# BenniG123/icp-slam-prototype

Hardware: AMD Instinct MI355X
Metric: ICP iterations/sec + NN Mpoints/sec at 307k-pt Kinect cloud, 1/2/4/8 GPU (higher is better)
Workload: dtype f32 filter + f64 exact pair arithmetic (reference float semantics), f64 reductions and solve; 1 GPU; kinect640x480_30pct: ONE frame pair, 91870 source x 92170 target points, 20 fixed ICP iterations per step from the pair's initial pose, solve=reference, nn=grid (BASELINE configs[1]); the N > 1 lines run configs[3] (64 such pairs) and scale against frame_batch (--full); parallelism=1 GPU

## Files before the change

icp_slam_prototype_amd/csrc/icpk_align.cpp:

```cpp
#include <chrono>
#include <cstring>
#include <utility>
#include <vector>

#include "icpk_ctx.h"
#include "solve_impl.h"

using namespace icpk;

namespace {

hipEvent_t get_event(icpk_ctx* ctx, size_t k) {
  while (ctx->events.size() <= k) {
    hipEvent_t e = nullptr;
    if (hipEventCreate(&e) != hipSuccess) return nullptr;
    ctx->events.push_back(e);
  }
  return ctx->events[k];
}

void log_delta(icpk_ctx* ctx, int key, int quantity) {
  if (!ctx->log_fn) return;
  const auto now = std::chrono::steady_clock::now();
  const double us = std::chrono::duration<double, std::micro>(now - ctx->log_last).count();
// ... 64 lines not shown

void pack_pose(float T_out[16], int solve, const float Trot[9], const float offset[3], const double Tk[12]) {
  if (solve == ICPK_SOLVE_REFERENCE) {
    for (int r = 0; r < 3; ++r) {
      for (int c = 0; c < 3; ++c) T_out[4 * r + c] = Trot[3 * r + c];
      T_out[4 * r + 3] = offset[r];
    }
  } else {
    for (int r = 0; r < 3; ++r)
      for (int c = 0; c < 4; ++c) T_out[4 * r + c] = (float)Tk[4 * r + c];
  }
  T_out[12] = T_out[13] = T_out[14] = 0.f;
  T_out[15] = 1.f;
}

int begin_alignment(icpk_ctx* ctx) {
  const int rc = copy_src0_to_src(ctx);
  if (rc) return rc;
  ctx->src_pristine = false;
  ctx->have_seed = false;
  ctx->have_qperm = false;
  clear_trace(ctx);
  return ICPK_OK;
}

}

namespace icpk {

int loop_nsum(const icpk_params* p) {
  if (p->solve == ICPK_SOLVE_POINT_TO_PLANE || p->solve == ICPK_SOLVE_PLANE_TO_PLANE) return NP2L;
  return p->solve == ICPK_SOLVE_REFERENCE ? NSUM_REF : NSUM;
}

int device_loop_begin(icpk_ctx* ctx, const icpk_params* p, bool throttled, bool mirror, bool defer) {
  LoopInitArgs a{};
  a.st = ctx->st_dev;
  if (throttled || mirror) {
    ctx->loop_epoch = (ctx->loop_epoch % 1000000) + 1;
    a.epoch = ctx->loop_epoch;
    a.progress = ctx->progress_dev;
    a.mirror = mirror ? ctx->st_mirror_dev : nullptr;
  }
  a.max_iterations = p->max_iterations;
  a.min_pairs = p->min_pairs;
  a.solve = p->solve;
  a.fixed_iterations = p->fixed_iterations;
  a.threshold = p->threshold;
  std::memcpy(a.last_rotation, p->last_rotation, sizeof(a.last_rotation));
  std::memcpy(a.last_translation, p->last_translation, sizeof(a.last_translation));
  if (defer) {
    ctx->pending_init = a;
    ctx->init_pending = true;
  } else {
    launch_loop_init(a, ctx->stream);
    ICPK_HIP(ctx, hipGetLastError());
  }
  const int nsum = loop_nsum(p);
// ... 156 lines not shown
  if (rc) return rc;
  if (!p || !T_out) return ICPK_E_ARG;
  if (p->nn_mode == ICPK_NN_MAP) return fail(ctx, ICPK_E_ARG, "ICPK_NN_MAP is single-context only");
  if (p->solve == ICPK_SOLVE_PLANE_TO_PLANE) return fail(ctx, ICPK_E_ARG, "the query-sharded loop has no plane-to-plane flavour");
  if (colored_step(ctx, p)) return fail(ctx, ICPK_E_ARG, "the query-sharded loop has no colored flavour (icpk_set_colored is on)");
  if (!ctx->comm) return fail(ctx, ICPK_E_NOT_SET, "icpk_comm_init_rccl has not been called");
  if (p->solve != ICPK_SOLVE_REFERENCE && p->solve != ICPK_SOLVE_KABSCH)
    return fail(ctx, ICPK_E_ARG, "the query-sharded loop supports the reference and Kabsch flavours");
  if (p->max_iterations < 0 || p->max_iterations > LOOP_MAX_ITER) return fail(ctx, ICPK_E_ARG, "max_iterations out of range");
  if (p->min_pairs < 1) return fail(ctx, ICPK_E_ARG, "min_pairs must be >= 1");
  if (ctx->robust_on) return fail(ctx, ICPK_E_ARG, "robust alignment is not available in the query-sharded loop");
  ICPK_HIP(ctx, hipSetDevice(ctx->device));
  reset_outputs(T_out, stats);
  icpk_params q = *p;
  q.nn_mode = ICPK_NN_GRID;
  rc = begin_alignment(ctx);
  if (rc) return rc;
  const LoopGuard guard{ctx};
  rc = device_loop_begin(ctx, &q, false);
  if (rc) return rc;
  ctx->loop_nact = NSUM;
  const int B = red_blocks(ctx->src.n);
  auto sweep = [&]() -> int {
    int r = enqueue_nn(ctx, ICPK_NN_GRID);
    if (r) return r;
    r = enqueue_reduce(ctx, q.max_nn_dist);
    if (r) return r;
    launch_reduce_final_shard(ctx->partial, ctx->pcount, B, ctx->red_out, ctx->st_dev, ctx->stream);
    return icpk_comm_allreduce_device(ctx, ctx->red_out, NSUM + 1);
  };
  rc = sweep();
// ... 28 lines not shown
  if (gicp && ctx->robust_on) return fail(ctx, ICPK_E_ARG, "plane-to-plane has no robust form (icpk_set_robust is on)");
  if (gicp && (!ctx->have_normals || !ctx->have_src_normals))
    return fail(ctx, ICPK_E_NOT_SET, "plane-to-plane needs source and target normals");
  const bool colored = colored_step(ctx, p);
  if (colored && ctx->robust_on) return fail(ctx, ICPK_E_ARG, "colored ICP has no robust form (icpk_set_robust is on)");
  if (colored && (!ctx->have_src_colors || !ctx->have_tgt_colors || !ctx->have_color_gradients))
    return fail(ctx, ICPK_E_NOT_SET, "colored ICP needs source colours, target colours and target colour gradients");
  if (ctx->robust_on && p->solve == ICPK_SOLVE_REFERENCE)
    return fail(ctx, ICPK_E_ARG, "robust alignment needs the Kabsch or point-to-plane flavour");
  int rc = check_ready(ctx);
  if (rc) {
    if (stats) stats->status = rc;
    return rc;
  }
  ICPK_HIP(ctx, hipSetDevice(ctx->device));
  rc = begin_alignment(ctx);
  if (rc) return rc;
  const bool robust = ctx->robust_on;
  if (robust && ctx->src.n > 0 && (rc = ensure_robust(ctx, ctx->src.n))) return rc;
  if (!p->host_loop && !ctx->log_fn && ctx->src.n > 0 && p->max_iterations <= LOOP_MAX_ITER)
    return align_device_loop(ctx, p, T_out, stats);

  Profiler pf(ctx, p);
  const bool p2l = p->solve == ICPK_SOLVE_POINT_TO_PLANE;
  const int nsum = robust ? (p2l ? NP2L_W : NSUM_W) : (p2l || gicp ? NP2L : NSUM);
  double Tk[12] = {1, 0, 0, 0, 0, 1, 0, 0, 0, 0, 1, 0};
  double sums[NSUM_MAX];
  int64_t npairs = 0, kept = 0;
  double wsum = 0.0;
  RobustSel sel{};
  float mse = 0.f;
  auto sweep = [&]() -> int {
    int r = pf.sweep(p->nn_mode);
    if (r) return r;
    r = pf.stamp(&pf.red);
    if (r) return r;
// ... 148 lines not shown
```

icp_slam_prototype_amd/csrc/icpk_api.cpp:

```cpp
#include <cmath>
#include <cstdlib>
#include <cstring>
#include <string>

#include "icpk_ctx.h"
#include "solve_impl.h"

using namespace icpk;

namespace {

int upload_cloud(icpk_ctx* ctx, Cloud& c, const float* x, const float* y, const float* z, int n, float pad,
                 hipMemcpyKind kind, bool sync = true) {
  if (n < 0 || (n > 0 && (!x || !y || !z))) return fail(ctx, ICPK_E_ARG, "bad cloud pointers/size");
  int rc = ensure_cloud(ctx, c, n);
  if (rc) return rc;
  if (n > 0 && kind == hipMemcpyHostToDevice && !sync) {
    PinnedBuf<float>& stage = (&c == &ctx->tgt) ? ctx->stage_t : ctx->stage_s;
    if ((rc = stage.reserve(ctx, (size_t)3 * c.cap))) return rc;
    std::memcpy(stage, x, (size_t)n * sizeof(float));
    std::memcpy(stage + c.cap, y, (size_t)n * sizeof(float));
    std::memcpy(stage + 2 * (size_t)c.cap, z, (size_t)n * sizeof(float));
    ICPK_HIP(ctx, hipMemcpyAsync(c.base, stage, ((size_t)2 * c.cap + n) * sizeof(float), hipMemcpyHostToDevice, ctx->stream));
  } else if (n > 0) {
// ... 121 lines not shown
  ICPK_HIP(ctx, hipSetDevice(ctx->device));
  int rc = upload_cloud(ctx, ctx->src0, x, y, z, n, 0.f, k, sync);
  if (rc) return rc;
  ctx->have_src = true;
  ctx->have_assoc = false;
  ctx->have_seed = false;
  ctx->have_qperm = false;
  return copy_src0_to_src(ctx);
}

int copy_src0_to_src(icpk_ctx* ctx) {
  ctx->rec_pending = false;
  if (ctx->src_pristine && ctx->tune.pristine_skip && ctx->src.n == ctx->src0.n) return ICPK_OK;
  int rc = ensure_cloud(ctx, ctx->src, ctx->src0.n);
  if (rc) return rc;
  const Cloud &a = ctx->src0, &b = ctx->src;
  if (a.cap == b.cap) {
    ICPK_HIP(ctx, hipMemcpyAsync(b.base, a.base, (size_t)3 * a.cap * sizeof(float), hipMemcpyDeviceToDevice, ctx->stream));
  } else {
    const int m = round_up(a.n < 1 ? 1 : a.n, NN_TILE);
    ICPK_HIP(ctx, hipMemcpyAsync(b.x(), a.x(), (size_t)m * sizeof(float), hipMemcpyDeviceToDevice, ctx->stream));
    ICPK_HIP(ctx, hipMemcpyAsync(b.y(), a.y(), (size_t)m * sizeof(float), hipMemcpyDeviceToDevice, ctx->stream));
    ICPK_HIP(ctx, hipMemcpyAsync(b.z(), a.z(), (size_t)m * sizeof(float), hipMemcpyDeviceToDevice, ctx->stream));
  }
  ctx->src_pristine = true;
  return ICPK_OK;
}

int check_ready(icpk_ctx* ctx) {
  if (!ctx) return ICPK_E_ARG;
  if (!ctx->have_tgt || !ctx->have_src) return fail(ctx, ICPK_E_NOT_SET, "source or target cloud not set");
  if (ctx->tgt.n <= 0) return fail(ctx, ICPK_E_EMPTY_TARGET, "target cloud is empty");
  return ICPK_OK;
}

int pad_target(icpk_ctx* ctx) {
  Cloud& c = ctx->tgt;
  const int padded = round_up(c.n < 1 ? 1 : c.n, NN_TILE);
  launch_fill_f32(c.x() + c.n, padded - c.n, __builtin_inff(), ctx->stream);
  launch_fill_f32(c.y() + c.n, padded - c.n, __builtin_inff(), ctx->stream);
// ... 306 lines not shown
```

icp_slam_prototype_amd/csrc/icpk_ctx.h:

```cpp
#pragma once
#include <hip/hip_runtime.h>

#include <chrono>
#include <string>
#include <thread>
#include <vector>

#include "icpk.h"
#include "icpk_internal.h"

struct icpk_ctx;

namespace icpk {

inline int hip_failure(icpk_ctx* ctx, const char* what, hipError_t e);

struct DeviceMem {
  static constexpr const char* name = "hipMalloc";
  static hipError_t alloc(void** p, size_t bytes) { return hipMalloc(p, bytes); }
  static hipError_t free(void* p) { return hipFree(p); }
};
template <unsigned Flags>
struct PinnedMem {
  static constexpr const char* name = "hipHostMalloc";
// ... 183 lines not shown
  int sub_factor = 0;
  unsigned long long sub_seed = 0;
  unsigned long long sub_stream = 0;
  struct HostRange {
    const char* host;
    size_t bytes;
    const char* dev;
  };
  std::vector<HostRange> registered;
  icpk::PinnedBuf<uint16_t> stage_depth;
  icpk::DevBuf<int> pix_tidx;
  icpk::DevBuf<int> pix_src;
  bool have_pix_seed = false;
  int pix_rows = 0, pix_cols = 0;
  bool src_pristine = false;
  const int* stop = nullptr;
  LoopState* st_active = nullptr;
  icpk::PinnedBuf<float> stage_t, stage_s;
  icpk::DevBuf<uint16_t> depth_dev;
  icpk::DevBuf<uint16_t> depth_flt;
  icpk::DevBuf<uint16_t> bil_tables;
  std::vector<uint16_t> bil_tables_host;
  icpk_bilateral_params bil_params = {0, 0.f, 0.f, 0};
  int bil_K = 0;
  icpk::DevBuf<int32_t> ks_buf;
  int frame_slot = -1;
  int frame_rows = 0, frame_cols = 0;
  int frame_filter[6] = {0, 0, 0, 0, 0, 0};
  icpk::DevBuf<int> bp_counts;
  icpk::PinnedBuf<int> bp_n_host;
// ... 186 lines not shown
    t_query = now + std::chrono::milliseconds(20);
    const hipError_t q = hipStreamQuery(stream ? stream : ctx->stream);
    if (q == hipSuccess) return done() ? ICPK_OK : fail(ctx, ICPK_E_HIP, stalled);
    if (q != hipErrorNotReady) return fail(ctx, ICPK_E_HIP, hipGetErrorString(q));
  }
  return ICPK_OK;
}

icpk_ctx* make_context(int device_id, const icpk_ctx* parent);
int check_ready(icpk_ctx* ctx);
int set_target_impl(icpk_ctx* ctx, const float* x, const float* y, const float* z, int32_t n, hipMemcpyKind k,
                    bool sync = true);
int set_source_impl(icpk_ctx* ctx, const float* x, const float* y, const float* z, int32_t n, hipMemcpyKind k,
                    bool sync = true);
int copy_src0_to_src(icpk_ctx* ctx);
int pad_target(icpk_ctx* ctx);
void target_changed(icpk_ctx* ctx, bool keep_normals);
void reset_outputs(float T_out[16], icpk_stats* stats);
void clear_trace(icpk_ctx* ctx);

int ensure_cloud(icpk_ctx* ctx, Cloud& c, int n);
int ensure_assoc(icpk_ctx* ctx, int nq);
int index_cloud(icpk_ctx* ctx, const float* x, const float* y, const float* z, int n, GridIndex& g);
int index_target(icpk_ctx* ctx, GridView* out);
int index_aux(icpk_ctx* ctx, const Cloud& c, GridView* out);
int ensure_unpacked(icpk_ctx* ctx);
int flush_loop_init(icpk_ctx* ctx);
NnArgs base_nn_args(const icpk_ctx* ctx);
int prepare_sorted_sweep(icpk_ctx* ctx, int nn_mode, NnArgs& a, NnBoxes& bx, int& recheck);
GridSweepArgs grid_sweep_args(icpk_ctx* ctx, const NnArgs& a, const NnBoxes& bx);
void after_grid_sweep(icpk_ctx* ctx);
int enqueue_nn(icpk_ctx* ctx, int nn_mode, hipEvent_t ev0 = nullptr, hipEvent_t ev1 = nullptr);
const float4* loop_rec(const icpk_ctx* ctx);
int enqueue_reduce(icpk_ctx* ctx, float max_dist);
int enqueue_reduce_p2l(icpk_ctx* ctx, float max_dist);
int enqueue_reduce_gicp(icpk_ctx* ctx, float max_dist, const float* R_acc);
int enqueue_reduce_colored(icpk_ctx* ctx, float max_dist);
inline bool colored_step(const icpk_ctx* ctx, const icpk_params* p) {
  return ctx->colored_on && p->solve == ICPK_SOLVE_POINT_TO_PLANE;
}
int ensure_robust(icpk_ctx* ctx, int nq);
// ... 18 lines not shown
```

icp_slam_prototype_amd/csrc/icpk_internal.h:

```cpp
#pragma once
#include <hip/hip_runtime.h>
#include <stddef.h>
#include <stdint.h>

#include "tsdf_rule.h"

namespace icpk {

constexpr int NN_THREADS = 256;
constexpr int NN_TILE = 1024;
static_assert(NN_TILE == 4 * NN_THREADS, "one float4 per lane per plane per tile");

typedef unsigned long long nn_key_t;
constexpr nn_key_t NN_KEY_INIT = ~0ull;

struct NnArgs {
  const float* qx;
  const float* qy;
  const float* qz;
  int nq;
  const float* tx;
  const float* ty;
  const float* tz;
  int nt_pad;
// ... 124 lines not shown
  int status;
  int sweeps;
  int steps;
  long long pairs;
  float mse;
  int epoch;
  int* progress;
  LoopState* mirror;
  Rt rt;
  double Rd[9];
  float Trot[9];
  float offset[3];
  double Tk[12];
  int max_iterations, min_pairs, solve, fixed_iterations;
  float threshold;
  float last_rotation[9], last_translation[3];
  float trace_R[LOOP_MAX_ITER * 9];
  float trace_t[LOOP_MAX_ITER * 3];
  float trace_mse[LOOP_MAX_ITER];
  int trace_pairs[LOOP_MAX_ITER];
};
__device__ __forceinline__ bool loop_stopped(const int* stop) { return stop && (stop[0] | stop[1]); }

struct StepArgs {
  const double* partial;
  const int* pcount;
  int nblocks;
  int pad0;
  LoopState* st;
};
// ... 176 lines not shown
  int n, n_pad;
  float pad;
  int cap1;
  float* d1;
  float* d2;
  int cap2;
  int pad0;
};
struct LoopInitArgs {
  LoopState* st;
  int* progress;
  LoopState* mirror;
  int max_iterations, min_pairs, solve, fixed_iterations;
  float threshold;
  int epoch;
  float last_rotation[9], last_translation[3];
};
struct BoundsArgs {
  const float *x, *y, *z;
  float* fb;
  int n, nparts;
};
struct InfoArgs {
  const float* fb;
  GridInfo* g;
  int nparts, n;
  float ppc;
  int xdiv;
  int max_cells;
  int pad0;
// ... 66 lines not shown
inline int grid_bounds_parts(int n) {
  const int nb = (n + 2047) / 2048;
  return nb < 1 ? 1 : (nb > GRID_BOUNDS_PARTS ? GRID_BOUNDS_PARTS : nb);
}
inline BoundsArgs bounds_args(const float* x, const float* y, const float* z, int n, float* fb) {
  return BoundsArgs{x, y, z, fb, n, grid_bounds_parts(n)};
}
inline InfoArgs info_args(const float* fb, int n, float ppc, int xdiv, int max_cells, GridInfo* g) {
  return InfoArgs{fb, g, grid_bounds_parts(n), n, ppc, xdiv < 1 ? 1 : xdiv, max_cells < 64 ? 64 : max_cells, 0};
}
void launch_ingest_cloud(const IngestArgs& a, hipStream_t s);
void launch_loop_init(const LoopInitArgs& a, hipStream_t s);
void launch_grid_bounds(const BoundsArgs& a, hipStream_t s);
void launch_grid_info(const InfoArgs& a, hipStream_t s);
void launch_grid_qslot(const QslotArgs& a, hipStream_t s);
void launch_grid_scan(const ScanArgs& a, hipStream_t s);
void launch_grid_tscatter(const TscatterArgs& a, hipStream_t s);
void launch_grid_qscatter(const QscatterArgs& a, hipStream_t s);
void launch_grid_begin(const BoundsArgs& a, const InfoArgs& info, const LoopInitArgs* init, int* ticket, hipStream_t s);
bool flush_setup_batches(const SetupRecorder* recs, int count, hipStream_t s);
void replay_setup(const SetupRecorder& rec, hipStream_t s);
void launch_ingest_batch(const SetupBatchOf<IngestArgs>& b, int count, hipStream_t s);
void launch_loop_init_batch(const SetupBatchOf<LoopInitArgs>& b, int count, hipStream_t s);
void launch_grid_bounds_batch(const SetupBatchOf<BoundsArgs>& b, int count, hipStream_t s);
void launch_grid_info_batch(const SetupBatchOf<InfoArgs>& b, int count, hipStream_t s);
void launch_grid_qslot_batch(const SetupBatchOf<QslotArgs>& b, int count, hipStream_t s);
void launch_grid_scan_batch(const SetupBatchOf<ScanArgs>& b, int count, hipStream_t s);
void launch_grid_tscatter_batch(const SetupBatchOf<TscatterArgs>& b, int count, hipStream_t s);
void launch_grid_qscatter_batch(const SetupBatchOf<QscatterArgs>& b, int count, hipStream_t s);
void launch_grid_tqscatter(const TscatterArgs& t, const QscatterArgs& q, hipStream_t s);
// ... 333 lines not shown
```

icp_slam_prototype_amd/csrc/icpk_sweep.cpp:

```cpp
#include <cstring>
#include <utility>

#include "icpk_ctx.h"

using namespace icpk;

namespace icpk {

int ensure_cloud(icpk_ctx* ctx, Cloud& c, int n) {
  if (ctx && (&c == &ctx->src0 || &c == &ctx->src)) ctx->src_pristine = false;
  if (ctx && &c == &ctx->src) ctx->rec_pending = false;
  if (ctx && &c == &ctx->src0) ctx->have_src_normals = false;
  if (ctx && &c == &ctx->src0) fpfh_dropped(ctx, 0);
  if (ctx && &c == &ctx->src0) ctx->have_src_colors = false;
  if (ctx && (&c == &ctx->src0 || &c == &ctx->tgt)) ctx->have_pix_seed = false;
  if (ctx && (&c == &ctx->src0 || &c == &ctx->tgt)) ctx->have_score_assoc = false;
  const int cap = round_up(n < 1 ? 1 : n, NN_TILE);
  if (cap > c.cap) {
    c.cap = 0;
    if (int rc = c.base.reserve(ctx, (size_t)3 * cap + 64)) return rc;
    c.cap = cap;
  }
  c.n = n;
  return ICPK_OK;
}

// ... 130 lines not shown
    ctx->have_grid = !rc;
  }
  if (!rc && out) *out = ctx->grid.view();
  return rc;
}

int index_aux(icpk_ctx* ctx, const Cloud& c, GridView* out) {
  if (c.n > (1 << 28)) return fail(ctx, ICPK_E_ARG, "the grid search addresses its cell-sorted points with 32-bit byte offsets: at most 2^28 points");
  int rc = ctx->aux_grid.reserve(ctx, c.n);
  if (!rc) rc = index_cloud(ctx, c.x(), c.y(), c.z(), c.n, ctx->aux_grid);
  if (!rc) *out = ctx->aux_grid.view();
  return rc;
}

static QscatterArgs query_scatter_args(icpk_ctx* ctx, const int* qcell, const int* qslot, float4* qm4, bool pix) {
  return QscatterArgs{qcell,        qslot,        ctx->qstart,  ctx->qperm, ctx->src.x(), ctx->src.y(), ctx->src.z(),
                      ctx->tgt.x(), ctx->tgt.y(), ctx->tgt.z(), qm4,        ctx->sp_in,   ctx->seed_m,  ctx->src.n,
                      0,            pix ? ctx->pix_src.get() : nullptr,     pix ? ctx->pix_tidx.get() : nullptr,
                      ctx->pix_rows, ctx->pix_cols};
}

static int enqueue_cell_order(icpk_ctx* ctx, bool with_points) {
  const int nq = ctx->src.n;
  int rc = ensure_sort_buffers(ctx, nq);
  if (rc) return rc;
  rc = ensure_scan_buffers(ctx);
  if (rc) return rc;
  int* qcell = reinterpret_cast<int*>(ctx->sort_keys + ctx->sort_cap);
  int* qslot = ctx->sort_vals;
  const bool ident = ctx->have_pix_seed && ctx->tune.image_order;
  const bool pix = ctx->have_pix_seed && ctx->tune.pixel_seeds && with_points;
  if (!ident) {
    ctx->qcount_dirty = true;
    launch_grid_qslot(QslotArgs{ctx->src.x(), ctx->src.y(), ctx->src.z(), ctx->grid.info, ctx->qcount, qcell, qslot, nq, 1},
                      ctx->stream);
    launch_grid_scan(ScanArgs{ctx->qcount, ctx->qstart, ctx->scan_bsum, ctx->grid.info, 1, 0}, ctx->stream);
  }
  launch_grid_qscatter(query_scatter_args(ctx, ident ? nullptr : qcell, qslot, with_points ? ctx->qm4.get() : nullptr, pix),
                       ctx->stream);
  ICPK_HIP(ctx, hipGetLastError());
  ctx->qcount_dirty = false;
  return ICPK_OK;
}

static int ensure_query_points(icpk_ctx* ctx, int nq);

int ensure_unpacked(icpk_ctx* ctx) {
  if (!ctx->rec_pending) return ICPK_OK;
  ctx->rec_pending = false;
  launch_grid_unpack(ctx->qm4, ctx->rec, ctx->src.n, ctx->src.x(), ctx->src.y(), ctx->src.z(), ctx->best, ctx->stream);
  ICPK_HIP(ctx, hipGetLastError());
  return ICPK_OK;
}

int flush_loop_init(icpk_ctx* ctx) {
  if (!ctx->init_pending) return ICPK_OK;
  ctx->init_pending = false;
  launch_loop_init(ctx->pending_init, ctx->stream);
  ICPK_HIP(ctx, hipGetLastError());
  return ICPK_OK;
}

// ... 25 lines not shown
  if (fresh) {
    const hipError_t e = hipMemsetAsync(ctx->grid_ticket, 0, sizeof(int), ctx->stream);
    if (e != hipSuccess) {
      (void)ctx->grid_ticket.release();
      return hip_failure(ctx, "hipMemsetAsync(grid_ticket)", e);
    }
  }
  GridIndex& g = ctx->grid;
  launch_grid_begin(bounds_args(ctx->tgt.x(), ctx->tgt.y(), ctx->tgt.z(), nt, g.bounds),
                    info_args(g.bounds, nt, ctx->tune.grid_ppc, ctx->tune.grid_xdiv, ctx->grid_max_cells, g.info),
                    ctx->init_pending ? &ctx->pending_init : nullptr, ctx->grid_ticket, ctx->stream);
  ctx->init_pending = false;
  ctx->qcount_dirty = ctx->qcount2_dirty = true;
  SetupBatchOf<QslotArgs> qb{};
  qb.p[0] = QslotArgs{ctx->tgt.x(), ctx->tgt.y(), ctx->tgt.z(), g.info, ctx->qcount, tcell, tslot, nt, 0};
  qb.p[1] = QslotArgs{ctx->src.x(), ctx->src.y(), ctx->src.z(), g.info, ctx->qcount2, qcell, qslot, nq, 1};
  const bool ident = ctx->have_pix_seed && ctx->tune.image_order;
  launch_grid_qslot_batch(qb, ident ? 1 : 2, ctx->stream);
  SetupBatchOf<ScanArgs> sb{};
  sb.p[0] = ScanArgs{ctx->qcount, g.cell_start, ctx->scan_bsum, g.info, 0, 0};
  sb.p[1] = ScanArgs{ctx->qcount2, ctx->qstart, ctx->scan_bsum2, g.info, 1, 0};
  launch_grid_scan_batch(sb, ident ? 1 : 2, ctx->stream);
  const TscatterArgs ta{ctx->tgt.x(), ctx->tgt.y(), ctx->tgt.z(), tcell, tslot, g.cell_start, g.t4, g.o4, nt, 0};
  const bool pix = ctx->have_pix_seed && ctx->tune.pixel_seeds;
  launch_grid_tqscatter(ta, query_scatter_args(ctx, ident ? nullptr : qcell, qslot, ctx->qm4, pix), ctx->stream);
  ICPK_HIP(ctx, hipGetLastError());
  ctx->qcount_dirty = ctx->qcount2_dirty = false;
  ctx->have_grid = true;
  return ICPK_OK;
}

// ... 61 lines not shown
  } else if (nn_mode == ICPK_NN_GRID) {
    if (!points_written) launch_fill_u64(ctx->seed_m, nq, 0ull, nullptr, ctx->stream);
    recheck = 1;
  } else {
    launch_seed_morton(ctx->sort_keys, ctx->qperm, nq, ctx->src.x(), ctx->src.y(), ctx->src.z(), ctx->tkeys,
                       ctx->sorted.x(), ctx->sorted.y(), ctx->sorted.z(), ctx->tperm, ctx->tgt.n, ctx->seed_m,
                       ctx->stream);
    recheck = 1;
  }
  a.tx = ctx->sorted.x();
  a.ty = ctx->sorted.y();
  a.tz = ctx->sorted.z();
  a.tiles_per_chunk = a.nt_pad / NN_TILE;
  a.best = ctx->best;
  if (nn_mode == ICPK_NN_GRID) {
    if (!(ctx->st_active && ctx->grid_chain) && !points_written)
      launch_grid_query_points(ctx->src.x(), ctx->src.y(), ctx->src.z(), ctx->qperm, nq, ctx->seed_m, bx.ox, bx.oy,
                               bx.oz, ctx->qm4, ctx->sp_in, ctx->stream);
  }
  ICPK_HIP(ctx, hipGetLastError());
  return ICPK_OK;
}

static int grid_slices_for(const icpk_ctx* ctx, int nq) { return ctx->tune.grid_slices ? ctx->tune.grid_slices : (nq > 524288 ? 4 : 8); }

GridSweepArgs grid_sweep_args(icpk_ctx* ctx, const NnArgs& a, const NnBoxes& bx) {
  GridSweepArgs g{};
  g.qx = const_cast<float*>(a.qx);
  g.qy = const_cast<float*>(a.qy);
  g.qz = const_cast<float*>(a.qz);
  g.nq = a.nq;
  g.qm4 = ctx->qm4;
  g.t4 = ctx->grid.t4;
// ... 394 lines not shown
```

icp_slam_prototype_amd/csrc/kernels_grid.hip:

```cpp
#include <type_traits>

#include "icpk_internal.h"
#include "loop_init.h"
#include "nn_device.h"
#include "wave_sum.h"

namespace icpk {

__device__ __forceinline__ void grid_bounds_body(const BoundsArgs& a, const int part) {
  __shared__ float red[6][16];
  float lo[3], hi[3];
#pragma unroll
  for (int c = 0; c < 3; ++c) {
    lo[c] = __builtin_inff();
    hi[c] = -__builtin_inff();
  }
  for (int i = part * 1024 + threadIdx.x; i < a.n; i += a.nparts * 1024) {
    const float v[3] = {a.x[i], a.y[i], a.z[i]};
#pragma unroll
    for (int c = 0; c < 3; ++c)
      if (v[c] - v[c] == 0.f) {
        lo[c] = __builtin_fminf(lo[c], v[c]);
        hi[c] = __builtin_fmaxf(hi[c], v[c]);
      }
// ... 108 lines not shown
  grid_info_body(a.fb, a.nparts, a.n, a.ppc, a.xdiv, a.max_cells, a.g);
}


__device__ __forceinline__ void grid_qslot_body(const QslotArgs& a, const int block) {
  const int i = block * blockDim.x + threadIdx.x;
  if (i >= a.n) return;
  const GridInfo g = *a.gi;
  const int cx = grid_cell(a.x[i], g.lo[0], g.inv_hx, g.nx);
  const int cy = grid_cell(a.y[i], g.lo[1], g.inv_h, g.ny);
  const int cz = grid_cell(a.z[i], g.lo[2], g.inv_h, g.nz);
  const int c = a.coarse ? (cz * g.ny + cy) * g.nxq + cx / g.xdiv : (cz * g.ny + cy) * g.nx + cx;
  a.cell[i] = c;
  a.slot[i] = atomicAdd(&a.count[c], 1);
}
__global__ void grid_qslot_kernel(const QslotArgs a) { grid_qslot_body(a, blockIdx.x); }
__global__ void grid_qslot_batch_kernel(const SetupBatchOf<QslotArgs> b) { grid_qslot_body(b.p[blockIdx.y], blockIdx.x); }

__device__ __forceinline__ void grid_qscatter_body(const QscatterArgs& a, const int block) {
  const int i = block * blockDim.x + threadIdx.x;
  if (i >= a.n) return;
  const int ip = a.qcell ? a.qstart[a.qcell[i]] + a.qslot[i] : i;
  a.qperm[ip] = i;
  if (a.qm4) {
    a.qm4[ip] = make_float4(a.qx[i], a.qy[i], a.qz[i], __int_as_float(i));
    int j = 0;
    if (a.spix) {
      const int p = a.spix[i];
      const int r = p / a.cols, c = p - r * a.cols;
      int found = a.tidx[p];
      auto ring_search = [&](auto ring_c) {
// ... 162 lines not shown
  for (int k = 0; k < count; ++k) m = b.p[k].n > m ? b.p[k].n : m;
  return m;
}

void launch_grid_tscatter(const TscatterArgs& a, hipStream_t s) {
  if (a.n <= 0 || record_setup_step(SK_TSCATTER, &SetupCall::tscatter, a)) return;
  hipLaunchKernelGGL(grid_tscatter_kernel, dim3((a.n + 255) / 256), dim3(256), 0, s, a);
}
void launch_grid_tscatter_batch(const SetupBatchOf<TscatterArgs>& b, int count, hipStream_t s) {
  const int m = max_n(b, count);
  if (count > 0 && m > 0) hipLaunchKernelGGL(grid_tscatter_batch_kernel, dim3((m + 255) / 256, count), dim3(256), 0, s, b);
}

void launch_grid_qslot(const QslotArgs& a, hipStream_t s) {
  if (a.n <= 0 || record_setup_step(SK_QSLOT, &SetupCall::qslot, a)) return;
  hipLaunchKernelGGL(grid_qslot_kernel, dim3((a.n + 255) / 256), dim3(256), 0, s, a);
}
void launch_grid_qslot_batch(const SetupBatchOf<QslotArgs>& b, int count, hipStream_t s) {
  const int m = max_n(b, count);
  if (count > 0 && m > 0) hipLaunchKernelGGL(grid_qslot_batch_kernel, dim3((m + 255) / 256, count), dim3(256), 0, s, b);
}
void launch_grid_qscatter(const QscatterArgs& a, hipStream_t s) {
  if (a.n <= 0 || record_setup_step(SK_QSCATTER, &SetupCall::qscatter, a)) return;
  hipLaunchKernelGGL(grid_qscatter_kernel, dim3((a.n + 255) / 256), dim3(256), 0, s, a);
}
void launch_grid_qscatter_batch(const SetupBatchOf<QscatterArgs>& b, int count, hipStream_t s) {
  const int m = max_n(b, count);
  if (count > 0 && m > 0) hipLaunchKernelGGL(grid_qscatter_batch_kernel, dim3((m + 255) / 256, count), dim3(256), 0, s, b);
}

__global__ void grid_tqscatter_kernel(const TscatterArgs t, const QscatterArgs q) {
// ... 473 lines not shown
```

icp_slam_prototype_amd/csrc/kernels_loop.hip:

```cpp
#include "icpk_internal.h"
#include "loop_init.h"
#include "solve_impl.h"
#include "pair_reduce.h"

namespace icpk {

#ifdef ICPK_STEP_STAMPS
__device__ unsigned long long step_dbg[8 * 64];
#define STEP_STAMP(i, k)                                                        \
  do {                                                                          \
    if (threadIdx.x == 0 && (i) < 64) step_dbg[(i) * 8 + (k)] = wall_clock64(); \
  } while (0)
extern "C" int icpk_debug_read_step_stamps(unsigned long long* out) {
  return (int)hipMemcpyFromSymbol(out, HIP_SYMBOL(step_dbg), sizeof(step_dbg));
}
#else
#define STEP_STAMP(i, k)
#endif

template <int NS, int NACT = NS>
__device__ __forceinline__ void tree_stage2(const double* __restrict__ partial, const int* __restrict__ pcount,
                                            int nblocks, double (&sums)[NS], long long& count) {
  const int tid = threadIdx.x;
  double v[NACT];
// ... 46 lines not shown
__device__ void compose_rt(const float Rf[9], const float tf[3], double Tk[12]) {
  double Tn[12];
  for (int r = 0; r < 3; ++r)
    for (int c = 0; c < 4; ++c) {
      double s = 0;
      for (int k = 0; k < 3; ++k) s += (double)Rf[3 * r + k] * Tk[4 * k + c];
      Tn[4 * r + c] = s + (c == 3 ? (double)tf[r] : 0.0);
    }
  for (int k = 0; k < 12; ++k) Tk[k] = Tn[k];
}

__device__ __forceinline__ void publish_progress(LoopState* __restrict__ st) {
  const int k = st->steps + 1;
  st->steps = k;
  int* pr = st->progress;
  if (pr) {
    const int e = st->epoch;
    __hip_atomic_store(pr + 1, (e << 2) | ((st->done != 0) << 1) | ((st->done | st->stop_after_transform) != 0), __ATOMIC_RELAXED,
                       __HIP_MEMORY_SCOPE_SYSTEM);
    __hip_atomic_store(pr, (e << 10) | k, __ATOMIC_RELAXED, __HIP_MEMORY_SCOPE_SYSTEM);
  }
}

__device__ __forceinline__ void publish_result(LoopState* __restrict__ st) {
  LoopState* __restrict__ m = st->mirror;
  if (!m) return;
  m->done = st->done;
  m->iterations = st->iterations;
  m->status = st->status;
  m->sweeps = st->sweeps;
  m->pairs = st->pairs;
  m->mse = st->mse;
  for (int k = 0; k < 9; ++k) m->Trot[k] = st->Trot[k];
  for (int k = 0; k < 3; ++k) m->offset[k] = st->offset[k];
  for (int k = 0; k < 12; ++k) m->Tk[k] = st->Tk[k];
  __hip_atomic_store(st->progress + 2, (st->epoch << 1) | 1, __ATOMIC_RELEASE, __HIP_MEMORY_SCOPE_SYSTEM);
}

template <int NS, int NACT = NS>
__device__ __forceinline__ void loop_step_body(const double* __restrict__ partial, const int* __restrict__ pcount,
                                               int nblocks, LoopState* __restrict__ st, int stats_only,
                                               const RobustSel* __restrict__ sel = nullptr,
                                               RobustTraceEntry* __restrict__ rtrace = nullptr) {
  constexpr bool ROBUST = NS == NSUM_W || NS == NP2L_W;
  constexpr bool P2L = NS == NP2L || NS == NP2L_W;
  const int done = st->done, stop_after = st->stop_after_transform, i = st->iterations;
  const int max_iterations = st->max_iterations, min_pairs = st->min_pairs, fixed = st->fixed_iterations;
  const float threshold = st->threshold;
  STEP_STAMP(i, 0);
  double sums[NS];
  long long npairs = 0;
  if (nblocks < 0) {
    if (threadIdx.x == 0) {
#pragma unroll
      for (int s = 0; s < NS; ++s) sums[s] = partial[s];
      npairs = (long long)(partial[NS] + 0.5);
    }
  } else {
    tree_stage2<NS, NACT>(partial, pcount, nblocks, sums, npairs);
  }
  STEP_STAMP(i, 1);
  if (done) {
    if (threadIdx.x == 0) publish_progress(st);
    return;
  }
  if (stop_after) {
    if (threadIdx.x == 0) {
      st->done = 1;
      publish_result(st);
      publish_progress(st);
    }
    return;
  }
  if (threadIdx.x != 0) return;

  float mse = 0.f;
  if (npairs > 0) {
    const float m = (float)(sums[P2L ? 27 : 12] / (double)npairs);
    mse = (float)((double)m * (double)m);
  }
  st->pairs = npairs;
  st->mse = mse;
  if (stats_only) {
    publish_result(st);
    return;
  }

  if (!((fixed || mse > threshold) && i < max_iterations)) {
    st->done = 1;
    publish_result(st);
    publish_progress(st);
    return;
  }
  const long long kept = ROBUST ? (long long)sums[NS - 1] : npairs;
  if (kept < min_pairs) {
    for (int k = 0; k < 9; ++k) st->rt.R[k] = st->last_rotation[k];
    for (int k = 0; k < 3; ++k) {
      st->rt.t[k] = st->last_translation[k];
      st->offset[k] = -st->last_translation[k];
    }
    for (int k = 0; k < 9; ++k) st->Rd[k] = (double)st->rt.R[k];
    st->status = 1;
    st->stop_after_transform = 1;
    publish_progress(st);
    return;
  }
  st->trace_pairs[i] = (int)npairs;
  st->trace_mse[i] = mse;
  LoopState* __restrict__ mir = st->mirror;
  if (mir) {
    mir->trace_pairs[i] = (int)npairs;
    mir->trace_mse[i] = mse;
  }
  if constexpr (ROBUST) {
    RobustTraceEntry e;
    e.kept = (int)kept;
    e.cut = sel->cut;
    e.c = sel->c;
    e.wsum = sums[NS - 2];
    rtrace[i] = e;
  }
  float Rrec[9], trec[3];
  STEP_STAMP(i, 2);
  if (P2L) {
    double Rd[9], td[3];
    if (!solve_p2l(sums, Rd, td)) {
      st->status = 2;
      st->done = 1;
      publish_result(st);
      publish_progress(st);
      return;
    }
    for (int k = 0; k < 9; ++k) Rrec[k] = (float)Rd[k];
    for (int k = 0; k < 3; ++k) trec[k] = (float)td[k];
    for (int k = 0; k < 9; ++k) st->rt.R[k] = Rrec[k];
    for (int k = 0; k < 3; ++k) st->rt.t[k] = trec[k];
    compose_rt(Rrec, trec, st->Tk);
  } else if (st->solve == 0) {
    float M[9], Rinv[9];
    for (int k = 0; k < 9; ++k) M[k] = (float)sums[k];
    solve_reference(M, Rrec);
    STEP_STAMP(i, 5);
    if (i == 0) {
      for (int k = 0; k < 9; ++k) st->Trot[k] = Rrec[k];
    } else {
      float tmp[9], cur[9];
// ... 15 lines not shown
      sb[k] = sums[16 + k];
    }
    for (int r = 0; r < 3; ++r)
      for (int c = 0; c < 3; ++c) sab[3 * r + c] = sums[3 * c + r];
    solve_kabsch(ROBUST ? sums[NS - 2] : (double)npairs, sa, sb, sab, Rd, td);
    for (int k = 0; k < 9; ++k) Rrec[k] = (float)Rd[k];
    for (int k = 0; k < 3; ++k) trec[k] = (float)td[k];
    for (int k = 0; k < 9; ++k) st->rt.R[k] = Rrec[k];
    for (int k = 0; k < 3; ++k) st->rt.t[k] = trec[k];
    compose_rt(Rrec, trec, st->Tk);
  }
  STEP_STAMP(i, 3);
  for (int k = 0; k < 9; ++k) st->Rd[k] = (double)st->rt.R[k];
  for (int k = 0; k < 9; ++k) st->trace_R[9 * i + k] = Rrec[k];
  for (int k = 0; k < 3; ++k) st->trace_t[3 * i + k] = trec[k];
  if (mir) {
    for (int k = 0; k < 9; ++k) mir->trace_R[9 * i + k] = Rrec[k];
    for (int k = 0; k < 3; ++k) mir->trace_t[3 * i + k] = trec[k];
  }
  st->iterations = i + 1;
  publish_progress(st);
  STEP_STAMP(i, 4);
}

template <int NS, int NACT = NS>
__global__ __launch_bounds__(256) void loop_step_kernel(const double* __restrict__ partial,
                                                        const int* __restrict__ pcount, int nblocks,
                                                        LoopState* __restrict__ st, int stats_only) {
  loop_step_body<NS, NACT>(partial, pcount, nblocks, st, stats_only);
}

template <int NS>
__global__ __launch_bounds__(256) void loop_step_robust_kernel(const double* __restrict__ partial,
                                                               const int* __restrict__ pcount, int nblocks,
                                                               LoopState* __restrict__ st, int stats_only,
                                                               const RobustSel* __restrict__ sel,
                                                               RobustTraceEntry* __restrict__ rtrace) {
// ... 83 lines not shown
```

icp_slam_prototype_amd/csrc/loop_init.h:

```cpp
#pragma once
#include <cstddef>

#include "icpk_internal.h"

namespace icpk {

__device__ __forceinline__ void loop_init_body(const LoopInitArgs& a) {
  constexpr int WORDS = (int)(offsetof(LoopState, trace_R) / 4);
  int* w = reinterpret_cast<int*>(a.st);
  for (int i = threadIdx.x; i < WORDS; i += blockDim.x) w[i] = 0;
  __syncthreads();
  if (threadIdx.x != 0) return;
  LoopState* st = a.st;
  st->Trot[0] = st->Trot[4] = st->Trot[8] = 1.f;
  st->Tk[0] = st->Tk[5] = st->Tk[10] = 1.0;
  st->max_iterations = a.max_iterations;
  st->min_pairs = a.min_pairs;
  st->solve = a.solve;
  st->fixed_iterations = a.fixed_iterations;
  st->threshold = a.threshold;
  st->epoch = a.epoch;
  st->progress = a.progress;
  st->mirror = a.mirror;
  for (int k = 0; k < 9; ++k) st->last_rotation[k] = a.last_rotation[k];
  for (int k = 0; k < 3; ++k) st->last_translation[k] = a.last_translation[k];
}

}
```

Baseline: 38350 iter/s.

## Defer source copy, fuse loop init into qslot, batch mirror publishing

Skips the per-alignment device copy of the pristine source planes by letting grid query kernels read directly from src0, copying lazily only when unpacking is needed. Folds the loop-state init into the first grid qslot launch to drop a kernel launch. Publishes progress only when throttled, and moves mirror trace writes out of every step into a wave-parallel copy at result time. This trims per-step system-scope stores and launches, at the cost of extra state (src_deferred) that must stay consistent across code paths.

```diff
diff --git a/icp_slam_prototype_amd/csrc/icpk_align.cpp b/icp_slam_prototype_amd/csrc/icpk_align.cpp
--- a/icp_slam_prototype_amd/csrc/icpk_align.cpp
+++ b/icp_slam_prototype_amd/csrc/icpk_align.cpp
@@ -102,8 +102,9 @@
   T_out[15] = 1.f;
 }
 
-int begin_alignment(icpk_ctx* ctx) {
-  const int rc = copy_src0_to_src(ctx);
+int begin_alignment(icpk_ctx* ctx, bool rec_loop) {
+  int rc = copy_src0_to_src(ctx);
+  if (!rc && !(rec_loop && ctx->src.n > 0)) rc = ensure_unpacked(ctx);
   if (rc) return rc;
   ctx->src_pristine = false;
   ctx->have_seed = false;
@@ -130,6 +131,7 @@
     a.progress = ctx->progress_dev;
     a.mirror = mirror ? ctx->st_mirror_dev : nullptr;
   }
+  a.throttled = throttled;
   a.max_iterations = p->max_iterations;
   a.min_pairs = p->min_pairs;
   a.solve = p->solve;
@@ -316,7 +318,7 @@
   reset_outputs(T_out, stats);
   icpk_params q = *p;
   q.nn_mode = ICPK_NN_GRID;
-  rc = begin_alignment(ctx);
+  rc = begin_alignment(ctx, false);
   if (rc) return rc;
   const LoopGuard guard{ctx};
   rc = device_loop_begin(ctx, &q, false);
@@ -375,12 +377,12 @@
     return rc;
   }
   ICPK_HIP(ctx, hipSetDevice(ctx->device));
-  rc = begin_alignment(ctx);
+  const bool device_loop = !p->host_loop && !ctx->log_fn && p->max_iterations <= LOOP_MAX_ITER;
+  rc = begin_alignment(ctx, device_loop && p->nn_mode == ICPK_NN_GRID);
   if (rc) return rc;
   const bool robust = ctx->robust_on;
   if (robust && ctx->src.n > 0 && (rc = ensure_robust(ctx, ctx->src.n))) return rc;
-  if (!p->host_loop && !ctx->log_fn && ctx->src.n > 0 && p->max_iterations <= LOOP_MAX_ITER)
-    return align_device_loop(ctx, p, T_out, stats);
+  if (device_loop && ctx->src.n > 0) return align_device_loop(ctx, p, T_out, stats);
 
   Profiler pf(ctx, p);
   const bool p2l = p->solve == ICPK_SOLVE_POINT_TO_PLANE;
diff --git a/icp_slam_prototype_amd/csrc/icpk_api.cpp b/icp_slam_prototype_amd/csrc/icpk_api.cpp
--- a/icp_slam_prototype_amd/csrc/icpk_api.cpp
+++ b/icp_slam_prototype_amd/csrc/icpk_api.cpp
@@ -159,16 +159,27 @@
   if (ctx->src_pristine && ctx->tune.pristine_skip && ctx->src.n == ctx->src0.n) return ICPK_OK;
   int rc = ensure_cloud(ctx, ctx->src, ctx->src0.n);
   if (rc) return rc;
+  ctx->src_pristine = true;
+  ctx->src_deferred = ctx->tune.pristine_skip;
+  return ctx->src_deferred ? ICPK_OK : copy_source_planes(ctx, false);
+}
+
+int copy_source_planes(icpk_ctx* ctx, bool tail_only) {
   const Cloud &a = ctx->src0, &b = ctx->src;
-  if (a.cap == b.cap) {
+  const int m = round_up(a.n < 1 ? 1 : a.n, NN_TILE);
+  if (tail_only) {
+    if (m == a.n) return ICPK_OK;
+    const size_t bytes = (size_t)(m - a.n) * sizeof(float);
+    ICPK_HIP(ctx, hipMemcpyAsync(b.x() + a.n, a.x() + a.n, bytes, hipMemcpyDeviceToDevice, ctx->stream));
+    ICPK_HIP(ctx, hipMemcpyAsync(b.y() + a.n, a.y() + a.n, bytes, hipMemcpyDeviceToDevice, ctx->stream));
+    ICPK_HIP(ctx, hipMemcpyAsync(b.z() + a.n, a.z() + a.n, bytes, hipMemcpyDeviceToDevice, ctx->stream));
+  } else if (a.cap == b.cap) {
     ICPK_HIP(ctx, hipMemcpyAsync(b.base, a.base, (size_t)3 * a.cap * sizeof(float), hipMemcpyDeviceToDevice, ctx->stream));
   } else {
-    const int m = round_up(a.n < 1 ? 1 : a.n, NN_TILE);
     ICPK_HIP(ctx, hipMemcpyAsync(b.x(), a.x(), (size_t)m * sizeof(float), hipMemcpyDeviceToDevice, ctx->stream));
     ICPK_HIP(ctx, hipMemcpyAsync(b.y(), a.y(), (size_t)m * sizeof(float), hipMemcpyDeviceToDevice, ctx->stream));
     ICPK_HIP(ctx, hipMemcpyAsync(b.z(), a.z(), (size_t)m * sizeof(float), hipMemcpyDeviceToDevice, ctx->stream));
   }
-  ctx->src_pristine = true;
   return ICPK_OK;
 }
 
diff --git a/icp_slam_prototype_amd/csrc/icpk_ctx.h b/icp_slam_prototype_amd/csrc/icpk_ctx.h
--- a/icp_slam_prototype_amd/csrc/icpk_ctx.h
+++ b/icp_slam_prototype_amd/csrc/icpk_ctx.h
@@ -221,6 +221,7 @@
   bool have_pix_seed = false;
   int pix_rows = 0, pix_cols = 0;
   bool src_pristine = false;
+  bool src_deferred = false;
   const int* stop = nullptr;
   LoopState* st_active = nullptr;
   icpk::PinnedBuf<float> stage_t, stage_s;
@@ -437,6 +438,7 @@
 int set_source_impl(icpk_ctx* ctx, const float* x, const float* y, const float* z, int32_t n, hipMemcpyKind k,
                     bool sync = true);
 int copy_src0_to_src(icpk_ctx* ctx);
+int copy_source_planes(icpk_ctx* ctx, bool tail_only);
 int pad_target(icpk_ctx* ctx);
 void target_changed(icpk_ctx* ctx, bool keep_normals);
 void reset_outputs(float T_out[16], icpk_stats* stats);
@@ -448,6 +450,7 @@
 int index_target(icpk_ctx* ctx, GridView* out);
 int index_aux(icpk_ctx* ctx, const Cloud& c, GridView* out);
 int ensure_unpacked(icpk_ctx* ctx);
+inline const icpk::Cloud& query_cloud(const icpk_ctx* ctx) { return ctx->src_deferred ? ctx->src0 : ctx->src; }
 int flush_loop_init(icpk_ctx* ctx);
 NnArgs base_nn_args(const icpk_ctx* ctx);
 int prepare_sorted_sweep(icpk_ctx* ctx, int nn_mode, NnArgs& a, NnBoxes& bx, int& recheck);
diff --git a/icp_slam_prototype_amd/csrc/icpk_internal.h b/icp_slam_prototype_amd/csrc/icpk_internal.h
--- a/icp_slam_prototype_amd/csrc/icpk_internal.h
+++ b/icp_slam_prototype_amd/csrc/icpk_internal.h
@@ -162,6 +162,7 @@
   double Tk[12];
   int max_iterations, min_pairs, solve, fixed_iterations;
   float threshold;
+  int throttled;
   float last_rotation[9], last_translation[3];
   float trace_R[LOOP_MAX_ITER * 9];
   float trace_t[LOOP_MAX_ITER * 3];
@@ -368,6 +369,7 @@
   int max_iterations, min_pairs, solve, fixed_iterations;
   float threshold;
   int epoch;
+  int throttled;
   float last_rotation[9], last_translation[3];
 };
 struct BoundsArgs {
@@ -464,6 +466,7 @@
 void launch_grid_bounds(const BoundsArgs& a, hipStream_t s);
 void launch_grid_info(const InfoArgs& a, hipStream_t s);
 void launch_grid_qslot(const QslotArgs& a, hipStream_t s);
+bool launch_grid_qslot_init(const QslotArgs& a, const LoopInitArgs& init, hipStream_t s);
 void launch_grid_scan(const ScanArgs& a, hipStream_t s);
 void launch_grid_tscatter(const TscatterArgs& a, hipStream_t s);
 void launch_grid_qscatter(const QscatterArgs& a, hipStream_t s);
diff --git a/icp_slam_prototype_amd/csrc/icpk_sweep.cpp b/icp_slam_prototype_amd/csrc/icpk_sweep.cpp
--- a/icp_slam_prototype_amd/csrc/icpk_sweep.cpp
+++ b/icp_slam_prototype_amd/csrc/icpk_sweep.cpp
@@ -10,6 +10,7 @@
 int ensure_cloud(icpk_ctx* ctx, Cloud& c, int n) {
   if (ctx && (&c == &ctx->src0 || &c == &ctx->src)) ctx->src_pristine = false;
   if (ctx && &c == &ctx->src) ctx->rec_pending = false;
+  if (ctx && (&c == &ctx->src0 || &c == &ctx->src)) ctx->src_deferred = false;
   if (ctx && &c == &ctx->src0) ctx->have_src_normals = false;
   if (ctx && &c == &ctx->src0) fpfh_dropped(ctx, 0);
   if (ctx && &c == &ctx->src0) ctx->have_src_colors = false;
@@ -170,7 +171,8 @@
 }
 
 static QscatterArgs query_scatter_args(icpk_ctx* ctx, const int* qcell, const int* qslot, float4* qm4, bool pix) {
-  return QscatterArgs{qcell,        qslot,        ctx->qstart,  ctx->qperm, ctx->src.x(), ctx->src.y(), ctx->src.z(),
+  const Cloud& q = query_cloud(ctx);
+  return QscatterArgs{qcell,        qslot,        ctx->qstart,  ctx->qperm, q.x(),        q.y(),        q.z(),
                       ctx->tgt.x(), ctx->tgt.y(), ctx->tgt.z(), qm4,        ctx->sp_in,   ctx->seed_m,  ctx->src.n,
                       0,            pix ? ctx->pix_src.get() : nullptr,     pix ? ctx->pix_tidx.get() : nullptr,
                       ctx->pix_rows, ctx->pix_cols};
@@ -188,8 +190,12 @@
   const bool pix = ctx->have_pix_seed && ctx->tune.pixel_seeds && with_points;
   if (!ident) {
     ctx->qcount_dirty = true;
-    launch_grid_qslot(QslotArgs{ctx->src.x(), ctx->src.y(), ctx->src.z(), ctx->grid.info, ctx->qcount, qcell, qslot, nq, 1},
-                      ctx->stream);
+    const Cloud& q = query_cloud(ctx);
+    const QslotArgs qa{q.x(), q.y(), q.z(), ctx->grid.info, ctx->qcount, qcell, qslot, nq, 1};
+    if (ctx->init_pending && launch_grid_qslot_init(qa, ctx->pending_init, ctx->stream))
+      ctx->init_pending = false;
+    else
+      launch_grid_qslot(qa, ctx->stream);
     launch_grid_scan(ScanArgs{ctx->qcount, ctx->qstart, ctx->scan_bsum, ctx->grid.info, 1, 0}, ctx->stream);
   }
   launch_grid_qscatter(query_scatter_args(ctx, ident ? nullptr : qcell, qslot, with_points ? ctx->qm4.get() : nullptr, pix),
@@ -202,6 +208,10 @@
 static int ensure_query_points(icpk_ctx* ctx, int nq);
 
 int ensure_unpacked(icpk_ctx* ctx) {
+  if (ctx->src_deferred) {
+    ctx->src_deferred = false;
+    if (int rc = copy_source_planes(ctx, ctx->rec_pending)) return rc;
+  }
   if (!ctx->rec_pending) return ICPK_OK;
   ctx->rec_pending = false;
   launch_grid_unpack(ctx->qm4, ctx->rec, ctx->src.n, ctx->src.x(), ctx->src.y(), ctx->src.z(), ctx->best, ctx->stream);
@@ -257,7 +267,8 @@
   ctx->qcount_dirty = ctx->qcount2_dirty = true;
   SetupBatchOf<QslotArgs> qb{};
   qb.p[0] = QslotArgs{ctx->tgt.x(), ctx->tgt.y(), ctx->tgt.z(), g.info, ctx->qcount, tcell, tslot, nt, 0};
-  qb.p[1] = QslotArgs{ctx->src.x(), ctx->src.y(), ctx->src.z(), g.info, ctx->qcount2, qcell, qslot, nq, 1};
+  const Cloud& q = query_cloud(ctx);
+  qb.p[1] = QslotArgs{q.x(), q.y(), q.z(), g.info, ctx->qcount2, qcell, qslot, nq, 1};
   const bool ident = ctx->have_pix_seed && ctx->tune.image_order;
   launch_grid_qslot_batch(qb, ident ? 1 : 2, ctx->stream);
   SetupBatchOf<ScanArgs> sb{};
@@ -349,9 +360,11 @@
   a.tiles_per_chunk = a.nt_pad / NN_TILE;
   a.best = ctx->best;
   if (nn_mode == ICPK_NN_GRID) {
-    if (!(ctx->st_active && ctx->grid_chain) && !points_written)
-      launch_grid_query_points(ctx->src.x(), ctx->src.y(), ctx->src.z(), ctx->qperm, nq, ctx->seed_m, bx.ox, bx.oy,
-                               bx.oz, ctx->qm4, ctx->sp_in, ctx->stream);
+    if (!(ctx->st_active && ctx->grid_chain) && !points_written) {
+      const Cloud& q = query_cloud(ctx);
+      launch_grid_query_points(q.x(), q.y(), q.z(), ctx->qperm, nq, ctx->seed_m, bx.ox, bx.oy, bx.oz, ctx->qm4, ctx->sp_in,
+                               ctx->stream);
+    }
   }
   ICPK_HIP(ctx, hipGetLastError());
   return ICPK_OK;
diff --git a/icp_slam_prototype_amd/csrc/kernels_grid.hip b/icp_slam_prototype_amd/csrc/kernels_grid.hip
--- a/icp_slam_prototype_amd/csrc/kernels_grid.hip
+++ b/icp_slam_prototype_amd/csrc/kernels_grid.hip
@@ -146,7 +146,10 @@
   a.cell[i] = c;
   a.slot[i] = atomicAdd(&a.count[c], 1);
 }
-__global__ void grid_qslot_kernel(const QslotArgs a) { grid_qslot_body(a, blockIdx.x); }
+__global__ void grid_qslot_kernel(const QslotArgs a, const LoopInitArgs li, const int has_init) {
+  if (has_init && blockIdx.x == 0) loop_init_body(li);
+  grid_qslot_body(a, blockIdx.x);
+}
 __global__ void grid_qslot_batch_kernel(const SetupBatchOf<QslotArgs> b) { grid_qslot_body(b.p[blockIdx.y], blockIdx.x); }
 
 __device__ __forceinline__ void grid_qscatter_body(const QscatterArgs& a, const int block) {
@@ -339,7 +342,12 @@
 
 void launch_grid_qslot(const QslotArgs& a, hipStream_t s) {
   if (a.n <= 0 || record_setup_step(SK_QSLOT, &SetupCall::qslot, a)) return;
-  hipLaunchKernelGGL(grid_qslot_kernel, dim3((a.n + 255) / 256), dim3(256), 0, s, a);
+  hipLaunchKernelGGL(grid_qslot_kernel, dim3((a.n + 255) / 256), dim3(256), 0, s, a, LoopInitArgs{}, 0);
+}
+bool launch_grid_qslot_init(const QslotArgs& a, const LoopInitArgs& init, hipStream_t s) {
+  if (a.n <= 0 || setup_recorder()) return false;
+  hipLaunchKernelGGL(grid_qslot_kernel, dim3((a.n + 255) / 256), dim3(256), 0, s, a, init, 1);
+  return true;
 }
 void launch_grid_qslot_batch(const SetupBatchOf<QslotArgs>& b, int count, hipStream_t s) {
   const int m = max_n(b, count);
diff --git a/icp_slam_prototype_amd/csrc/kernels_loop.hip b/icp_slam_prototype_amd/csrc/kernels_loop.hip
--- a/icp_slam_prototype_amd/csrc/kernels_loop.hip
+++ b/icp_slam_prototype_amd/csrc/kernels_loop.hip
@@ -84,7 +84,7 @@
   const int k = st->steps + 1;
   st->steps = k;
   int* pr = st->progress;
-  if (pr) {
+  if (pr && st->throttled) {
     const int e = st->epoch;
     __hip_atomic_store(pr + 1, (e << 2) | ((st->done != 0) << 1) | ((st->done | st->stop_after_transform) != 0), __ATOMIC_RELAXED,
                        __HIP_MEMORY_SCOPE_SYSTEM);
@@ -95,23 +95,34 @@
 __device__ __forceinline__ void publish_result(LoopState* __restrict__ st) {
   LoopState* __restrict__ m = st->mirror;
   if (!m) return;
-  m->done = st->done;
-  m->iterations = st->iterations;
-  m->status = st->status;
-  m->sweeps = st->sweeps;
-  m->pairs = st->pairs;
-  m->mse = st->mse;
-  for (int k = 0; k < 9; ++k) m->Trot[k] = st->Trot[k];
-  for (int k = 0; k < 3; ++k) m->offset[k] = st->offset[k];
-  for (int k = 0; k < 12; ++k) m->Tk[k] = st->Tk[k];
-  __hip_atomic_store(st->progress + 2, (st->epoch << 1) | 1, __ATOMIC_RELEASE, __HIP_MEMORY_SCOPE_SYSTEM);
-}
-
-template <int NS, int NACT = NS>
-__device__ __forceinline__ void loop_step_body(const double* __restrict__ partial, const int* __restrict__ pcount,
-                                               int nblocks, LoopState* __restrict__ st, int stats_only,
-                                               const RobustSel* __restrict__ sel = nullptr,
-                                               RobustTraceEntry* __restrict__ rtrace = nullptr) {
+  const int lane = threadIdx.x, it = st->iterations;
+  if (lane == 0) {
+    m->done = st->done;
+    m->iterations = it;
+    m->status = st->status;
+    m->sweeps = st->sweeps;
+    m->pairs = st->pairs;
+    m->mse = st->mse;
+    for (int k = 0; k < 9; ++k) m->Trot[k] = st->Trot[k];
+    for (int k = 0; k < 3; ++k) m->offset[k] = st->offset[k];
+    for (int k = 0; k < 12; ++k) m->Tk[k] = st->Tk[k];
+  }
+  for (int k = lane; k < it; k += 64) {
+    m->trace_pairs[k] = st->trace_pairs[k];
+    m->trace_mse[k] = st->trace_mse[k];
+  }
+  for (int k = lane; k < 9 * it; k += 64) m->trace_R[k] = st->trace_R[k];
+  for (int k = lane; k < 3 * it; k += 64) m->trace_t[k] = st->trace_t[k];
+  __builtin_amdgcn_fence(__ATOMIC_RELEASE, "");
+  if (lane == 0) __hip_atomic_store(st->progress + 2, (st->epoch << 1) | 1, __ATOMIC_RELAXED, __HIP_MEMORY_SCOPE_SYSTEM);
+}
+
+enum : int { PUB_RESULT = 1, PUB_PROGRESS = 2 };
+
+template <int NS, int NACT = NS>
+__device__ __forceinline__ int loop_step_decide(const double* __restrict__ partial, const int* __restrict__ pcount,
+                                                int nblocks, LoopState* __restrict__ st, int stats_only,
+                                                const RobustSel* __restrict__ sel, RobustTraceEntry* __restrict__ rtrace) {
   constexpr bool ROBUST = NS == NSUM_W || NS == NP2L_W;
   constexpr bool P2L = NS == NP2L || NS == NP2L_W;
   const int done = st->done, stop_after = st->stop_after_transform, i = st->iterations;
@@ -130,19 +141,12 @@
     tree_stage2<NS, NACT>(partial, pcount, nblocks, sums, npairs);
   }
   STEP_STAMP(i, 1);
-  if (done) {
-    if (threadIdx.x == 0) publish_progress(st);
-    return;
-  }
+  if (threadIdx.x != 0) return 0;
+  if (done) return PUB_PROGRESS;
   if (stop_after) {
-    if (threadIdx.x == 0) {
-      st->done = 1;
-      publish_result(st);
-      publish_progress(st);
-    }
-    return;
-  }
-  if (threadIdx.x != 0) return;
+    st->done = 1;
+    return PUB_RESULT | PUB_PROGRESS;
+  }
 
   float mse = 0.f;
   if (npairs > 0) {
@@ -151,16 +155,11 @@
   }
   st->pairs = npairs;
   st->mse = mse;
-  if (stats_only) {
-    publish_result(st);
-    return;
-  }
+  if (stats_only) return PUB_RESULT;
 
   if (!((fixed || mse > threshold) && i < max_iterations)) {
     st->done = 1;
-    publish_result(st);
-    publish_progress(st);
-    return;
+    return PUB_RESULT | PUB_PROGRESS;
   }
   const long long kept = ROBUST ? (long long)sums[NS - 1] : npairs;
   if (kept < min_pairs) {
@@ -172,16 +171,10 @@
     for (int k = 0; k < 9; ++k) st->Rd[k] = (double)st->rt.R[k];
     st->status = 1;
     st->stop_after_transform = 1;
-    publish_progress(st);
-    return;
+    return PUB_PROGRESS;
   }
   st->trace_pairs[i] = (int)npairs;
   st->trace_mse[i] = mse;
-  LoopState* __restrict__ mir = st->mirror;
-  if (mir) {
-    mir->trace_pairs[i] = (int)npairs;
-    mir->trace_mse[i] = mse;
-  }
   if constexpr (ROBUST) {
     RobustTraceEntry e;
     e.kept = (int)kept;
@@ -197,9 +190,7 @@
     if (!solve_p2l(sums, Rd, td)) {
       st->status = 2;
       st->done = 1;
-      publish_result(st);
-      publish_progress(st);
-      return;
+      return PUB_RESULT | PUB_PROGRESS;
     }
     for (int k = 0; k < 9; ++k) Rrec[k] = (float)Rd[k];
     for (int k = 0; k < 3; ++k) trec[k] = (float)td[k];
@@ -245,13 +236,21 @@
   for (int k = 0; k < 9; ++k) st->Rd[k] = (double)st->rt.R[k];
   for (int k = 0; k < 9; ++k) st->trace_R[9 * i + k] = Rrec[k];
   for (int k = 0; k < 3; ++k) st->trace_t[3 * i + k] = trec[k];
-  if (mir) {
-    for (int k = 0; k < 9; ++k) mir->trace_R[9 * i + k] = Rrec[k];
-    for (int k = 0; k < 3; ++k) mir->trace_t[3 * i + k] = trec[k];
-  }
   st->iterations = i + 1;
-  publish_progress(st);
   STEP_STAMP(i, 4);
+  return PUB_PROGRESS;
+}
+
+template <int NS, int NACT = NS>
+__device__ __forceinline__ void loop_step_body(const double* __restrict__ partial, const int* __restrict__ pcount,
+                                               int nblocks, LoopState* __restrict__ st, int stats_only,
+                                               const RobustSel* __restrict__ sel = nullptr,
+                                               RobustTraceEntry* __restrict__ rtrace = nullptr) {
+  const int mine = loop_step_decide<NS, NACT>(partial, pcount, nblocks, st, stats_only, sel, rtrace);
+  if (threadIdx.x >= 64) return;
+  const int what = __builtin_amdgcn_readfirstlane(mine);
+  if (what & PUB_RESULT) publish_result(st);
+  if (threadIdx.x == 0 && (what & PUB_PROGRESS)) publish_progress(st);
 }
 
 template <int NS, int NACT = NS>
diff --git a/icp_slam_prototype_amd/csrc/loop_init.h b/icp_slam_prototype_amd/csrc/loop_init.h
--- a/icp_slam_prototype_amd/csrc/loop_init.h
+++ b/icp_slam_prototype_amd/csrc/loop_init.h
@@ -19,6 +19,7 @@
   st->solve = a.solve;
   st->fixed_iterations = a.fixed_iterations;
   st->threshold = a.threshold;
+  st->throttled = a.throttled;
   st->epoch = a.epoch;
   st->progress = a.progress;
   st->mirror = a.mirror;
```

After: 39780 iter/s, median of 6. +3.7%, better.
